# adobe/3D-FM-GAN

Hardware: AMD Instinct MI355X
Metric: (photo,render) pairs/sec (higher is better)
Workload: dtype f32; 1 GPU; pairs1024: cfg4 shard: E_Tsr+E_W+E_W_Plus(18 styles) on 256^2 -> co-mod -> Generator(1024) forward, fp32, B=8/GPU; pairs_per_gpu=8, global_pairs=8, image_size=1024, parallelism=replicas x1 (batch-sharded, no collective), launch=eager, ranks=1, full=False

## Files before the change

### 3d-fm-gan_amd/csrc/conv3x3_x3.hip

```cpp
#include "bf16_mfma.h"

namespace {

enum { C3_NONE = 0, C3_LRELU = 1, C3_PRELU = 2 };

struct C3Params {
  const float* in; const unsigned short* wt; const float* aux; float* out;
  int batch, cin, cout, h, w, oh, ow;
  int tiles_x, tiles_y, o_tiles, mp;
  float alpha;
  int stride, epi;
  int in_nhwc, out_nhwc;
};

template <int S>
struct C3Tile {
  static constexpr int BM = 64, TH = 4, TW = 32;
  static constexpr int PH = S * (TH - 1) + 3, PWP = S * (TW - 1) + 3, EVEN = (PWP + 1) / 2;
  static constexpr int PLANE = PH * PWP;
  static constexpr size_t LDS = (size_t)(3 * 2 * PLANE) * 16;
  static constexpr int BLOCKS_PER_CU = S == 1 ? 3 : 2;
};

bool c3_plan(C3Params& p) {
  if (p.batch <= 0 || p.cin <= 0 || p.cout <= 0 || p.h <= 0 || p.w <= 0) return false;
  if (p.stride != 1 && p.stride != 2) return false;
  if (p.in_nhwc && (p.cin & 3)) return false;
  using Tile = C3Tile<1>;
  p.oh = (p.h - 1) / p.stride + 1; p.ow = (p.w - 1) / p.stride + 1;
  p.mp = (p.cout + 31) / 32 * 32;
  p.tiles_x = (p.ow + Tile::TW - 1) / Tile::TW;
  p.tiles_y = (p.oh + Tile::TH - 1) / Tile::TH;
  p.o_tiles = (p.cout + Tile::BM - 1) / Tile::BM;
  if ((long long)p.cin * p.h * p.w * 4 >= 0xFFFFFFF0LL) return false;
  if ((long long)((p.cin + 15) / 16) * 54 * p.mp * 16 >= 0xFFFFFFF0LL) return false;
  if ((long long)p.o_tiles * p.tiles_x * p.tiles_y * p.batch > 0x7fffffffLL) return false;
  if ((long long)p.batch * p.cout * p.oh * p.ow > (1LL << 40)) return false;
  return true;
}

template <int S, bool NHWC_IN, int EPI>
__global__ __launch_bounds__(256, C3Tile<S>::BLOCKS_PER_CU) void conv3x3_mfma_bf16x3(const C3Params p) {
  using Tile = C3Tile<S>;
  constexpr int BM = Tile::BM, TH = Tile::TH, TW = Tile::TW, PWP = Tile::PWP, EVEN = Tile::EVEN, PLANE = Tile::PLANE;
  constexpr int RNP = 2;
  constexpr bool QUAD = NHWC_IN && S == 2;
  constexpr int NU = QUAD ? (4 * PLANE + 255) / 256 : (PLANE + 255) / 256, NV = QUAD ? 4 : 16;
  static_assert(NU <= 16, "one staging unit per issue_x call");
  extern __shared__ u32x4 smem_q[];
  u32x4* Xs = smem_q;

  const int tid = threadIdx.x, lane = tid & 63, wave = __builtin_amdgcn_readfirstlane(tid >> 6);
  const int l31 = lane & 31, khalf = lane >> 5, wm = wave & 1, wn = wave >> 1;
  const int kq = tid & 3;
  unsigned lb = xcd_remap(blockIdx.x, gridDim.x);
  const int o_tile = lb % p.o_tiles; lb /= p.o_tiles;
  const int tx_i = lb % p.tiles_x; lb /= p.tiles_x;
  const int ty_i = lb % p.tiles_y;
  const int b = lb / p.tiles_y;
  const int o0 = o_tile * BM, x0 = tx_i * TW, y0 = ty_i * TH;
  const int hw = p.h * p.w;
  const float* in_b = p.in + (long long)b * p.cin * hw;

  f32x16 acc[RNP], acc_lo[RNP];
#pragma unroll
  for (int g = 0; g < RNP; ++g)
#pragma unroll
    for (int r = 0; r < 16; ++r) { acc[g][r] = 0.f; acc_lo[g][r] = 0.f; }

  constexpr unsigned PARK = 0xFFFFFFF0u;
  const unsigned x_bytes = (unsigned)((long long)p.cin * hw * 4);
  const unsigned mp16 = (unsigned)p.mp * 16u;
  const unsigned w_bytes = (unsigned)((p.cin + 15) >> 4) * 54u * mp16;
  const auto rsrc_x = __builtin_amdgcn_make_buffer_rsrc(const_cast<float*>(in_b), 0, x_bytes, 0x00020000);
  const auto rsrc_w = __builtin_amdgcn_make_buffer_rsrc(const_cast<unsigned short*>(p.wt), 0, w_bytes, 0x00020000);
  unsigned xvo[NU];
#pragma unroll
  for (int u = 0; u < NU; ++u) {
    const int q = QUAD ? (tid + 256 * u) >> 2 : tid + 256 * u;
    const int r = q / PWP, t = q - r * PWP;
    const int c = S == 1 ? t : (t < EVEN ? 2 * t : 2 * (t - EVEN) + 1);
    const int y = S * y0 + r - 1, x = S * x0 + c - 1;
    const bool inside = q < PLANE && y >= 0 && y < p.h && x >= 0 && x < p.w;
    const unsigned pos_bytes = NHWC_IN ? 4u * (unsigned)p.cin : 4u;
    xvo[u] = inside ? (unsigned)(y * p.w + x) * pos_bytes + (QUAD ? 16u * (unsigned)kq : 0u) : PARK;
  }
  const int arow = o0 + wm * 32 + l31;
  const unsigned avo = arow < p.mp ? (unsigned)(khalf * p.mp + arow) * 16u : PARK;

  float xv[NU][NV];
  auto issue_x = [&](int i0, int kc) {
    if constexpr (QUAD) {
      if (kc < NU) {
// ... 44 lines not shown
          dst[0] = ph; dst[4 * PLANE] = pm; dst[8 * PLANE] = pl;
        }
      }
    } else {
      if (i0 + 16 > p.cin) {
#pragma unroll
        for (int kc = 0; kc < 16; ++kc)
          if (i0 + kc >= p.cin) {
#pragma unroll
            for (int u = 0; u < NU; ++u) xv[u][kc] = 0.f;
          }
      }
#pragma unroll
      for (int u = 0; u < NU; ++u) {
        const int q = tid + 256 * u;
        if (q < PLANE) {
#pragma unroll
          for (int hh = 0; hh < 2; ++hh) {
            unsigned h[4], m[4], l[4];
#pragma unroll
            for (int e = 0; e < 4; ++e) split2(xv[u][8 * hh + 2 * e], xv[u][8 * hh + 2 * e + 1], h[e], m[e], l[e]);
            u32x4 ph = {h[0], h[1], h[2], h[3]}, pm = {m[0], m[1], m[2], m[3]}, pl = {l[0], l[1], l[2], l[3]};
            Xs[(0 * 2 + hh) * PLANE + q] = ph;
            Xs[(1 * 2 + hh) * PLANE + q] = pm;
            Xs[(2 * 2 + hh) * PLANE + q] = pl;
          }
        }
      }
    }
  };

  int pbase[RNP];
#pragma unroll
  for (int g = 0; g < RNP; ++g) pbase[g] = khalf * PLANE + S * (wn * RNP + g) * PWP + l31;

  struct Ops { u32x4 a[3]; bf16x8 b[3][RNP]; };
  auto fetch_a = [&](Ops& o, unsigned soff_chunk, int t) {
#pragma unroll
    for (int pc = 0; pc < 3; ++pc)
      o.a[pc] = __builtin_bit_cast(u32x4, __builtin_amdgcn_raw_buffer_load_b128(rsrc_w, avo, soff_chunk + (unsigned)(pc * 18 + t * 2) * mp16, 0));
  };
  auto fetch_b = [&](Ops& o, int t) {
    const int ky = t / 3, kx = t - 3 * ky;
    const int off = S == 1 ? ky * PWP + kx : ky * PWP + (kx & 1) * EVEN + (kx >> 1);
#pragma unroll
    for (int pc = 0; pc < 3; ++pc)
#pragma unroll
      for (int g = 0; g < RNP; ++g) o.b[pc][g] = __builtin_bit_cast(bf16x8, Xs[pc * 2 * PLANE + pbase[g] + off]);
  };
  unsigned wflag = 0;

  const int chunks = (p.cin + 15) >> 4;
#pragma unroll
  for (int kc = 0; kc < 16; ++kc) issue_x(0, kc);
  for (int ch = 0; ch < chunks; ++ch) {
    const unsigned soff_chunk = (unsigned)ch * 54u * mp16;
    Ops ops[2];
    fetch_a(ops[0], soff_chunk, 0);
    __syncthreads();
    commit_x(16 * ch);
    __syncthreads();
    __builtin_amdgcn_sched_barrier(0);
    fetch_b(ops[0], 0);
    const int i0n = ch + 1 < chunks ? 16 * (ch + 1) : 0;
#pragma unroll
    for (int t = 0; t < 9; ++t) {
      __builtin_amdgcn_sched_barrier(0);
      if (t + 1 < 9) {
        fetch_a(ops[(t + 1) & 1], soff_chunk, t + 1);
        __builtin_amdgcn_sched_barrier(0);
        issue_x(i0n, 2 * t); issue_x(i0n, 2 * t + 1);
        fetch_b(ops[(t + 1) & 1], t + 1);
      }
      __builtin_amdgcn_sched_barrier(0);
      const Ops& o = ops[t & 1];
#pragma unroll
      for (int e = 0; e < 4; ++e) wflag |= ((o.a[0][e] & 0x7f807f80u) + 0x00800080u) & 0x80008000u;
      __builtin_amdgcn_s_setprio(1);
#pragma unroll
      for (int q = 0; q < 6; ++q)
#pragma unroll
        for (int g = 0; g < RNP; ++g) {
          f32x16& dst = q == 5 ? acc[g] : acc_lo[g];
          dst = __builtin_amdgcn_mfma_f32_32x32x16_bf16(__builtin_bit_cast(bf16x8, o.a[PA[q]]), o.b[PB[q]][g], dst, 0, 0, 0);
        }
      __builtin_amdgcn_s_setprio(0);
    }
    __builtin_amdgcn_sched_barrier(0);
  }
#pragma unroll
  for (int g = 0; g < RNP; ++g)
#pragma unroll
    for (int r = 0; r < 16; ++r) acc[g][r] = __fadd_rn(acc[g][r], acc_lo[g][r]);

  float* out_b = p.out + (long long)b * p.cout * p.oh * p.ow;
  const float alpha = p.alpha;
  auto epilogue = [&](float v, float a) -> float {
    if constexpr (EPI == C3_LRELU) {
      const float t = __fadd_rn(v, a);
      return t > 0.f ? t : t * alpha;
    } else if constexpr (EPI == C3_PRELU) {
      return v > 0.f ? v : a * v;
    } else {
      return v;
    }
  };
  const long long ost_o = p.out_nhwc ? 1 : (long long)p.oh * p.ow, ost_p = p.out_nhwc ? p.cout : 1;
  if (__syncthreads_or((xflag != xflag) | (wflag != 0u))) {
    const int pp = tid & 127, oy = y0 + (pp >> 5), ox = x0 + (pp & 31);
    if (oy >= p.oh || ox >= p.ow) return;
    for (int oo = 0; oo < 32; ++oo) {
      const int o = o0 + (tid >> 7) * 32 + oo;
      if (o >= p.cout) return;
      float s = 0.f;
      for (int i = 0; i < p.cin; ++i) {
        const long long slot0 = (long long)(i >> 4) * 54 * p.mp;
        const int hh = (i >> 3) & 1, j = i & 7;
        for (int t = 0; t < 9; ++t) {
          const int y = S * oy + t / 3 - 1, x = S * ox + t % 3 - 1;
          const long long at = NHWC_IN ? (long long)(y * p.w + x) * p.cin + i : (long long)i * hw + y * p.w + x;
          const float xin = (y >= 0 && y < p.h && x >= 0 && x < p.w) ? in_b[at] : 0.f;
          float wv = 0.f;
#pragma unroll
          for (int pc = 0; pc < 3; ++pc)
            wv += bf16_to_f32(p.wt[((slot0 + (long long)(pc * 18 + t * 2 + hh) * p.mp + o) << 3) + j]);
          s = __builtin_fmaf(wv, xin, s);
        }
      }
      out_b[o * ost_o + ((long long)oy * p.ow + ox) * ost_p] = epilogue(s, (EPI != C3_NONE && p.aux) ? p.aux[o] : 0.f);
    }
    return;
  }

  const int orow = o0 + wm * 32 + 4 * khalf;
  float aux_r[16];
#pragma unroll
  for (int r = 0; r < 16; ++r)
    aux_r[r] = (EPI != C3_NONE && p.aux) ? p.aux[min(orow + (r & 3) + 8 * (r >> 2), p.cout - 1)] : 0.f;
#pragma unroll
  for (int g = 0; g < RNP; ++g) {
    const int py_ = y0 + wn * RNP + g, px_ = x0 + l31;
    if (py_ >= p.oh || px_ >= p.ow) continue;
    float* dpos = out_b + ((long long)py_ * p.ow + px_) * ost_p;
    float v[16];
#pragma unroll
    for (int r = 0; r < 16; ++r) v[r] = epilogue(acc[g][r], aux_r[r]);
    if (p.out_nhwc && (p.cout & 3) == 0) {
#pragma unroll
      for (int j = 0; j < 4; ++j) {
        const int o = orow + 8 * j;
        if (o < p.cout) {
          f32x4 q4 = {v[4 * j], v[4 * j + 1], v[4 * j + 2], v[4 * j + 3]};
          *reinterpret_cast<f32x4*>(dpos + o) = q4;
        }
      }
    } else {
#pragma unroll
      for (int r = 0; r < 16; ++r) {
        const int o = orow + (r & 3) + 8 * (r >> 2);
        if (o < p.cout) dpos[o * ost_o] = v[r];
      }
    }
  }
}

template <int S, bool NHWC_IN, int EPI>
int c3_launch(const C3Params& p, hipStream_t s) {
  using Tile = C3Tile<S>;
  void (*kernel)(const C3Params) = conv3x3_mfma_bf16x3<S, NHWC_IN, EPI>;
  static bool opted_in = false;
  opt_in_dynamic_lds(kernel, Tile::LDS, opted_in);
  const long long blocks = (long long)p.o_tiles * p.tiles_x * p.tiles_y * p.batch;
  hipLaunchKernelGGL(kernel, dim3((unsigned)blocks), dim3(256), Tile::LDS, s, p);
  return fmgan_check_launch();
}

template <int S, bool NHWC_IN>
int c3_launch_epi(const C3Params& p, hipStream_t s) {
  if (p.epi == C3_LRELU) return c3_launch<S, NHWC_IN, C3_LRELU>(p, s);
  if (p.epi == C3_PRELU) return c3_launch<S, NHWC_IN, C3_PRELU>(p, s);
  return c3_launch<S, NHWC_IN, C3_NONE>(p, s);
}

int conv3x3_bf16x3(const float* in, const void* wt, const float* aux, float* out, int batch, int cin, int cout, int h, int w,
                   int stride, int in_nhwc, int out_nhwc, int epi, float alpha, hipStream_t s) {
  if (batch < 0 || cin <= 0 || cout <= 0 || h <= 0 || w <= 0 || (stride != 1 && stride != 2)) return FMGAN_EINVAL;
  if ((in_nhwc != 0 && in_nhwc != 1) || (out_nhwc != 0 && out_nhwc != 1) || epi < C3_NONE || epi > C3_PRELU) return FMGAN_EINVAL;
  if (batch == 0) return FMGAN_OK;
  C3Params p{};
  p.in = in; p.wt = (const unsigned short*)wt; p.aux = aux; p.out = out;
  p.batch = batch; p.cin = cin; p.cout = cout; p.h = h; p.w = w; p.alpha = alpha;
  p.stride = stride; p.epi = epi; p.in_nhwc = in_nhwc; p.out_nhwc = out_nhwc;
  if (!c3_plan(p)) return FMGAN_EUNSUPPORTED;
  if (!in || !wt || !out || (epi == C3_PRELU && !aux)) return FMGAN_EINVAL;
  if (in_nhwc && ((uintptr_t)in & 15)) return FMGAN_EINVAL;
  if (out_nhwc && (cout & 3) == 0 && ((uintptr_t)out & 15)) return FMGAN_EINVAL;
  if (stride == 1) return in_nhwc ? c3_launch_epi<1, true>(p, s) : c3_launch_epi<1, false>(p, s);
  return in_nhwc ? c3_launch_epi<2, true>(p, s) : c3_launch_epi<2, false>(p, s);
}

}

extern "C" int fmgan_conv3x3s2_bf16x3_supported(int batch, int cin, int cout, int h, int w) {
  return fmgan_conv3x3_bf16x3_supported(batch, cin, cout, h, w, 2, 0);
}

extern "C" int fmgan_conv3x3s2_bf16x3_f32(const float* in, const void* wt_split, const float* bias, float* out, int batch,
                                          int cin, int cout, int h, int w, float alpha, int out_nhwc, void* stream) {
  return conv3x3_bf16x3(in, wt_split, bias, out, batch, cin, cout, h, w, 2, 0, out_nhwc, C3_LRELU, alpha, (hipStream_t)stream);
}

extern "C" int fmgan_conv3x3_bf16x3_supported(int batch, int cin, int cout, int h, int w, int stride, int in_nhwc) {
  C3Params p{};
  p.batch = batch; p.cin = cin; p.cout = cout; p.h = h; p.w = w; p.stride = stride; p.in_nhwc = in_nhwc;
  return c3_plan(p) ? 1 : 0;
}

extern "C" int fmgan_conv3x3_bf16x3_f32(const float* in, const void* wt_split, const float* aux, float* out, int batch,
                                        int cin, int cout, int h, int w, int stride, int in_nhwc, int out_nhwc,
                                        int epilogue, float alpha, void* stream) {
  return conv3x3_bf16x3(in, wt_split, aux, out, batch, cin, cout, h, w, stride, in_nhwc, out_nhwc, epilogue, alpha,
                        (hipStream_t)stream);
}
```

### 3d-fm-gan_amd/op/_native/__init__.py

```python
from .core import (
    LIB_PATH, F32, F64, F16, BF16, FMGAN_OK, FMGAN_EINVAL, FMGAN_EUNSUPPORTED, amp_fwd, amp_bwd, lib, check, served,
    require_gpu, dtype_code, ptr, fp, require_f32_gpu, on_device, nhwc_dense, set_observer, launching)
from .activation import (
    activation_io, current_activation_io, io16, amp_fwd_io, BLUR_PATHS, upfirdn2d_out_size, upfirdn2d,
    upfirdn2d_strided, blur_noise_bias_act_serves, blur_noise_bias_act, fused_bias_act, fused_bias_act_backward,
    noise_bias_act, prelu_backward, dtype16_code, upfirdn2d16, fused_bias_act16, fused_bias_act16_backward)
from .conv import (
    modconv_demod, modconv_wsq, modconv_weight_prep, aligned_rows_shape, aligned_rows_buffer, modconv_precision,
    current_modconv_precision, modconv2d, modconv2d_rgb_fusable, modconv2d_select, modconv2d_tiles, modconv2d_rgb,
    modconv_weight_to_bf16, modconv_weight_to_bf16x3, conv_weight_to_bf16x3, conv3x3s2_bf16x3_supported,
    conv3x3s2_bf16x3, conv3x3_bf16x3_supported, conv3x3_bf16x3, C3_EPILOGUES, modconv_wgrad, wino_weight,
    wino_input, wino_output, modconv2d_winograd, torgb,
    torgb_backward, equal_linear, style_bank, style_bank_concat, demod_bank)
from .encoder import bn_prelu, se_pool, se_gate, ir_tail
from .loss import (
    LPIPS_SIZE, face_region_loss, face_region_loss_backward, render_mask, lpips_distance, lpips_distance_backward,
    lpips_pair_input, projection_loss_fwd, projection_loss_bwd, HEATMAP_SIZE, face_crop_serves, face_crop_fwd,
    face_crop_bwd, detector_input, heatmap_distance_serves, heatmap_distance_fwd, heatmap_distance_bwd,
    landmark_decode)
from .evaluation import (
    face_input_pool, face_input, f64p, fid_stats_serves, fid_stats_update, fid_stats_finish, INCEPTION_SIZE,
    inception_input)
from .image import (
    images_to_tensor, resize_output_size, resize_plan, resize_images, tensor_to_images, tiles_to_canvas,
    BANK_GATHER_BANKS, BANK_GATHER_GROUPS, bank_gather)
from .optim import (
    lbfgs_segments, lbfgs_pair, lbfgs_coeffs, lbfgs_direction, lbfgs_update, lbfgs_gather, EMA_CHUNK,
    LOSS_ROW_COLUMNS, ema_blocks, ema, loss_row)
```

### 3d-fm-gan_amd/op/_native/conv.py

```python
import ctypes

import torch

from .core import ambient, check, fp, launching, lib, nhwc_dense, _noise_args, on_device, ptr, require_gpu, served


def modconv_demod(weight, style, scale, eps=1e-8, wsq=None):
    cout, cin, kh, kw = weight.shape[-4:]
    style = style.contiguous()
    demod = torch.empty((style.shape[0], cout), dtype=torch.float32, device=style.device)
    with on_device(style) as stream:
        if wsq is not None:
            check(lib().fmgan_modconv_demod_wsq_f32(fp(wsq), fp(style), fp(demod), style.shape[0], cout, cin,
                                                    float(scale), float(eps), stream), 'modconv_demod_wsq')
        else:
            check(lib().fmgan_modconv_demod_f32(fp(weight), fp(style), fp(demod), style.shape[0], cout, cin,
                                                kh * kw, float(scale), float(eps), stream), 'modconv_demod')
    return demod


def modconv_wsq(weight):
    cout, cin, kh, kw = weight.shape[-4:]
    wsq = torch.empty((cout, cin), dtype=torch.float32, device=weight.device)
    with on_device(weight) as stream:
# ... 100 lines not shown
    rgb = torch.empty((b, rgb_c, h, w), dtype=torch.float32, device=x.device)
    nz, nb = _noise_args(noise)
    sk = rgb_skip.contiguous() if rgb_skip is not None else None
    wmod = torch.empty((b, 3, cout), dtype=torch.float32, device=x.device)
    with on_device(x) as stream:
        check(lib().fmgan_torgb_weight_mod_f32(fp(rgb_weight), fp(rgb_style), fp(wmod), b, cout, rgb_c,
                                               float(rgb_scale), stream), 'torgb_weight_mod')
    with launching(x, 'modconv2d', (b, cin, cout, h, w, 0)) as stream:
        st = lib().fmgan_modconv2d_rgb_f32(fp(x), fp(wt), fp(style), fp(demod), fp(out), b, cin, cout, h, w,
                                           fp(nz), fp(noise_weight), fp(bias), nb, 1, float(alpha), float(act_scale),
                                           fp(wmod), fp(rgb_bias), fp(sk), fp(rgb), rgb_c, stream)
    check(st, 'modconv2d_rgb')
    return out, rgb


def modconv_weight_to_bf16(wt):
    cin, taps, cout = wt.shape
    nbytes = lib().fmgan_modconv_weight_bf16_bytes(cin, cout, taps)
    wtb = torch.empty(nbytes // 2, dtype=torch.int16, device=wt.device)
    with on_device(wt) as stream:
        check(lib().fmgan_modconv_weight_to_bf16(fp(wt), ptr(wtb), cin, cout, taps, stream), 'modconv_weight_to_bf16')
    return wtb


def modconv_weight_to_bf16x3(wt):
    cin, taps, cout = wt.shape
    nbytes = lib().fmgan_modconv_weight_bf16x3_bytes(cin, cout, taps)
    wts = torch.empty(nbytes // 2, dtype=torch.int16, device=wt.device)
    with on_device(wt) as stream:
        check(lib().fmgan_modconv_weight_to_bf16x3(fp(wt), ptr(wts), cin, cout, taps, stream), 'modconv_weight_to_bf16x3')
    return wts


def conv_weight_to_bf16x3(weight):
    require_gpu(weight, 'weight')
    cout, cin, kh, kw = weight.shape
    with launching(weight, 'conv_weight_bf16x3', (cout, cin, kh * kw)):
        wt = weight.detach().permute(1, 2, 3, 0).reshape(cin, kh * kw, cout).contiguous()
        return modconv_weight_to_bf16x3(wt)


def conv3x3s2_bf16x3_supported(batch, cin, cout, h, w):
    return bool(lib().fmgan_conv3x3s2_bf16x3_supported(int(batch), int(cin), int(cout), int(h), int(w)))


def conv3x3s2_bf16x3(x, wts, bias, cout, alpha=0.01, channels_last=False):
    require_gpu(x, 'input')
    in_nhwc = _c3_input_layout('conv3x3s2_bf16x3', x)
    b, cin, h, w = x.shape
    out = torch.empty((b, cout, (h - 1) // 2 + 1, (w - 1) // 2 + 1), dtype=torch.float32, device=x.device,
                      memory_format=torch.channels_last if channels_last else torch.contiguous_format)
    with launching(x, 'conv3x3s2_bf16x3', (b, cin, cout, h, w)) as stream:
        if in_nhwc:
            st = lib().fmgan_conv3x3_bf16x3_f32(fp(x), ptr(wts), fp(bias), fp(out), b, cin, cout, h, w, 2, 1,
                                                int(bool(channels_last)), C3_EPILOGUES['lrelu'], float(alpha), stream)
        else:
            st = lib().fmgan_conv3x3s2_bf16x3_f32(fp(x), ptr(wts), fp(bias), fp(out), b, cin, cout, h, w, float(alpha),
                                                  int(bool(channels_last)), stream)
    return out if served(st, 'conv3x3s2_bf16x3') else None


C3_EPILOGUES = {None: 0, 'lrelu': 1, 'prelu': 2}


def _c3_input_layout(what, x):
    if x.is_contiguous():
        return 0
    if nhwc_dense(x):
        return 1
    raise RuntimeError(f'{what}: input must be NCHW-contiguous or dense channels_last, got strides {x.stride()}')


def conv3x3_bf16x3_supported(batch, cin, cout, h, w, stride=1, channels_last_in=False):
    return bool(lib().fmgan_conv3x3_bf16x3_supported(int(batch), int(cin), int(cout), int(h), int(w), int(stride),
                                                     int(bool(channels_last_in))))


def conv3x3_bf16x3(x, wts, cout, stride=1, epilogue=None, aux=None, alpha=0.01, channels_last=False):
    require_gpu(x, 'input')
    in_nhwc = _c3_input_layout('conv3x3_bf16x3', x)
    epi = C3_EPILOGUES[epilogue]
    if epilogue == 'prelu' and (aux is None or aux.numel() != cout):
        raise RuntimeError('conv3x3_bf16x3: the prelu epilogue needs one slope per output channel')
    if aux is not None:
        aux = aux.contiguous()
    stride = int(stride)
    b, cin, h, w = x.shape
    out = torch.empty((b, cout, (h - 1) // max(stride, 1) + 1, (w - 1) // max(stride, 1) + 1), dtype=torch.float32,
                      device=x.device, memory_format=torch.channels_last if channels_last else torch.contiguous_format)
    with launching(x, 'conv3x3_bf16x3', (b, cin, cout, h, w, stride, epi)) as stream:
        st = lib().fmgan_conv3x3_bf16x3_f32(fp(x), ptr(wts), fp(aux), fp(out), b, cin, cout, h, w, stride, in_nhwc,
                                            int(bool(channels_last)), epi, float(alpha), stream)
    return out if served(st, 'conv3x3_bf16x3') else None


def modconv_wgrad(go, demod, x, style, scale, fast_only=False, mode=0):
    go, x, style = go.contiguous(), x.contiguous(), style.contiguous()
    b, cout = go.shape[:2]
    cin, h, w = x.shape[1:]
    if (fast_only or mode != 0) and (cin < 48 or cout < 48):
        return None
    ws_bytes = lib().fmgan_modconv_wgrad_mode_workspace_bytes(b, cin, cout, h, w, int(mode))
    if ws_bytes == 0:
        return None
    ws = torch.empty(ws_bytes // 4, dtype=torch.float32, device=x.device)
    gw = torch.empty((cout, cin, 3, 3), dtype=torch.float32, device=x.device)
    with launching(x, 'modconv_wgrad', (b, cin, cout, h, w, int(mode))) as stream:
        st = lib().fmgan_modconv_wgrad_mode_f32(fp(go), fp(demod), fp(x), fp(style), fp(gw), b, cin, cout, h, w,
                                                int(mode), float(scale), fp(ws), ws_bytes, stream)
    check(st, 'modconv_wgrad')
    return gw


def wino_weight(wt):
    cin, taps, cout = wt.shape
    if taps != 9:
        raise RuntimeError('wino_weight: 3x3 weights only')
    u = torch.empty((16, cout, cin), dtype=torch.float32, device=wt.device)
    with on_device(wt) as stream:
        check(lib().fmgan_wino_weight_f32(fp(wt), fp(u), cin, cout, stream), 'wino_weight')
    return u


def wino_input(x, style):
    require_gpu(x, 'input')
    x, style = x.contiguous(), style.contiguous()
# ... 118 lines not shown
```

### 3d-fm-gan_amd/op/_native/core.py

```python
import ctypes
import os

import torch

_PKG = os.path.dirname(os.path.dirname(os.path.dirname(os.path.abspath(__file__))))
LIB_PATH = os.environ.get('FMGAN_LIB') or os.path.join(_PKG, 'csrc', 'libfmgan_hip.so')

F32, F64, F16 = 0, 1, 2
BF16 = 3
FMGAN_OK, FMGAN_EINVAL, FMGAN_EUNSUPPORTED = 0, -1, -2
_DTYPES = {torch.float32: F32, torch.float64: F64, torch.float16: F16}

_lib = None

amp_fwd = torch.amp.custom_fwd(device_type='cuda', cast_inputs=torch.float32)
amp_bwd = torch.amp.custom_bwd(device_type='cuda')


class ambient:
    values, text, scope, var = (), '', None, ''

    def __init__(self, value):
        if value not in self.values:
            raise ValueError(self.text)
# ... 38 lines not shown
    _sig(L.fmgan_noise_bias_act_f32, [vp] * 5 + [i] * 4 + [f, f, vp])
    _sig(L.fmgan_fused_bias_act_bwd_blocks, [ll, i])
    _sig(L.fmgan_fused_bias_act_bwd_f32, [vp] * 4 + [ll, i, f, f, vp])
    _sig(L.fmgan_prelu_backward_blocks, [ll, i])
    _sig(L.fmgan_prelu_backward_f32, [vp] * 5 + [ll, i, vp])
    _sig(L.fmgan_act16_fba_select, [i, ll, i, i, i, i])
    _sig(L.fmgan_act16_fba, [i, vp, vp, vp, vp, ll, i, i, i, i, f, f, vp])
    _sig(L.fmgan_act16_fba_bwd_blocks, [ll, i])
    _sig(L.fmgan_act16_fba_bwd, [i] + [vp] * 4 + [ll, i, f, f, vp])
    _sig(L.fmgan_ufd16_select, [i] * 15)
    _sig(L.fmgan_ufd16, [i, vp, vp, vp] + [i] * 14 + [vp])
    _sig(L.fmgan_modconv_demod_f32, [vp] * 3 + [i] * 4 + [f, f, vp])
    _sig(L.fmgan_modconv_wsq_f32, [vp] * 2 + [i] * 3 + [vp])
    _sig(L.fmgan_modconv_demod_wsq_f32, [vp] * 3 + [i] * 3 + [f, f, vp])
    _sig(L.fmgan_modconv_weight_prep_f32, [vp, vp, i, i, i, f, i, vp])
    _sig(L.fmgan_modconv2d_workspace_bytes, [i] * 6, ll)
    _sig(L.fmgan_modconv2d_f32, [vp] * 5 + [i] * 6 + [vp] * 3 + [i, i, f, f, ll, i, vp, ll, vp])
    _sig(L.fmgan_modconv2d_rgb_fusable, [i] * 5)
    _sig(L.fmgan_modconv2d_select, [i] * 8 + [ctypes.POINTER(i)] * 5)
    _sig(L.fmgan_modconv2d_tiles, [ctypes.POINTER(i), i])
    _sig(L.fmgan_modconv2d_rgb_f32, [vp] * 5 + [i] * 5 + [vp] * 3 + [i, i, f, f] + [vp] * 4 + [i, vp])
    _sig(L.fmgan_modconv_weight_bf16_bytes, [i] * 3, ll)
    _sig(L.fmgan_modconv_weight_to_bf16, [vp, vp, i, i, i, vp])
    _sig(L.fmgan_modconv2d_bf16_supported, [i] * 6)
    _sig(L.fmgan_modconv2d_bf16, [vp] * 5 + [i] * 6 + [vp] * 3 + [i, i, f, f, ll, i, vp])
    _sig(L.fmgan_modconv_weight_bf16x3_bytes, [i] * 3, ll)
    _sig(L.fmgan_modconv_weight_to_bf16x3, [vp, vp, i, i, i, vp])
    _sig(L.fmgan_modconv2d_bf16x3_supported, [i] * 6)
    _sig(L.fmgan_modconv2d_bf16x3, [vp] * 5 + [i] * 6 + [vp] * 3 + [i, i, f, f, ll, i, vp])
    _sig(L.fmgan_conv3x3s2_bf16x3_supported, [i] * 5)
    _sig(L.fmgan_conv3x3s2_bf16x3_f32, [vp] * 4 + [i] * 5 + [f, i, vp])
    _sig(L.fmgan_conv3x3_bf16x3_supported, [i] * 7)
    _sig(L.fmgan_conv3x3_bf16x3_f32, [vp] * 4 + [i] * 9 + [f, vp])
    _sig(L.fmgan_modconv_wgrad_workspace_bytes, [i] * 5, ll)
    _sig(L.fmgan_modconv_wgrad_f32, [vp] * 5 + [i] * 5 + [f, vp, ll, vp])
    _sig(L.fmgan_modconv_wgrad_mode_workspace_bytes, [i] * 6, ll)
    _sig(L.fmgan_modconv_wgrad_mode_f32, [vp] * 5 + [i] * 6 + [f, vp, ll, vp])
    _sig(L.fmgan_wino_weight_f32, [vp, vp, i, i, vp])
    _sig(L.fmgan_wino_input_f32, [vp] * 3 + [i] * 4 + [vp])
    _sig(L.fmgan_wino_output_f32, [vp] * 6 + [i] * 6 + [f, f, vp])
    _sig(L.fmgan_torgb_weight_mod_f32, [vp] * 3 + [i] * 3 + [f, vp])
    _sig(L.fmgan_torgb_f32, [vp] * 6 + [i] * 4 + [f, vp])
    _sig(L.fmgan_torgb_backward_splits, [i] * 3)
    _sig(L.fmgan_torgb_backward_f32, [vp] * 6 + [i] * 4 + [f, vp])
    _sig(L.fmgan_equal_linear_f32, [vp] * 4 + [i] * 3 + [vp])
    _sig(L.fmgan_style_bank_entry_bytes, [])
    _sig(L.fmgan_style_bank_f32, [vp, i, vp, vp, i, i, i, vp, vp])
    _sig(L.fmgan_style_bank_concat_f32, [vp, i, vp, vp, i, i, i, i, vp, vp])
    _sig(L.fmgan_demod_bank_f32, [vp, i, vp, i, vp, vp])
    _sig(L.fmgan_weight_refresh_blocks, [i, i, i, i, ll], ll)
    _sig(L.fmgan_weight_refresh_f32, [vp, i, ll, vp])
    _sig(L.fmgan_bn_prelu_f32, [vp] * 5 + [f, vp, vp] + [vp] * 4 + [f, vp, vp] + [i] * 5 + [vp])
    _sig(L.fmgan_se_pool_chunks, [i] * 4)
    _sig(L.fmgan_se_pool_f32, [vp, vp] + [i] * 4 + [vp])
    _sig(L.fmgan_se_gate_f32, [vp, i, ll] + [vp] * 4 + [f] + [vp] * 3 + [i] * 3 + [vp])
    _sig(L.fmgan_ir_tail_f32, [vp] * 5 + [f, vp, vp] + [i] * 3 + [vp] * 4 + [f, vp] + [vp] * 4 + [f, vp] + [i] * 4 + [vp])
    _sig(L.fmgan_face_region_blocks, [i, ll])
    _sig(L.fmgan_face_region_loss_f32, [vp] * 3 + [i, i, ll, vp])
    _sig(L.fmgan_face_region_backward_f32, [vp] * 4 + [i, i, ll, vp])
    _sig(L.fmgan_render_mask_f32, [vp] * 2 + [i, i, ll, vp])
    _sig(L.fmgan_lpips_distance_blocks, [i] * 3)
    _sig(L.fmgan_lpips_distance_f32, [vp] * 4 + [i, i, i, f, vp])
    _sig(L.fmgan_lpips_distance_backward_f32, [vp] * 6 + [i, i, i, f, vp])
    _sig(L.fmgan_lpips_pair_input_select, [i] * 8)
    _sig(L.fmgan_lpips_pair_input_f32, [vp] * 5 + [i] * 8 + [vp])
    _sig(L.fmgan_projection_loss_select, [i] * 4)
# ... 160 lines not shown
```

### 3d-fm-gan_amd/op/live_weights.py

```python
import weakref

import numpy as np
import torch

from . import _native

_ENTRY = np.dtype([('src', '<u8'), ('dst', '<u8'), ('dst2', '<u8'), ('n', '<i8'), ('kind', '<i4'), ('cout', '<i4'),
                   ('cin', '<i4'), ('ktaps', '<i4'), ('scale', '<f4'), ('block_begin', '<u4')])


def _check_layout():
    if _native.lib().fmgan_refresh_entry_bytes() != _ENTRY.itemsize:
        raise RuntimeError('fmgan_refresh_entry layout mismatch between libfmgan_hip.so and op/live_weights.py')


class LiveWeights:

    def __init__(self, root):
        self.root = root
        self.active = False
        self._key = None
        self._table = None
        self._blocks = 0
        self._n = 0
# ... 67 lines not shown
            _native.check(_native.lib().fmgan_weight_refresh_f32(self._table.data_ptr(), self._n, self._blocks, stream),
                          'weight_refresh')
        return True

    def fresh(self):
        return _Fresh(self)


class _Fresh:
    def __init__(self, lw):
        self.lw = lw

    def __enter__(self):
        self.prev = self.lw.active
        if not self.prev:
            self.lw.active = self.lw.refresh()
        return self.lw

    def __exit__(self, *exc):
        self.lw.active = self.prev
        return False


def live(module):
    lv = getattr(module, '_live', None)
    if lv is not None and lv[0].active and not torch.is_grad_enabled():
        return lv[1], lv[2]
    return None


_SPLIT = weakref.WeakKeyDictionary()


def split_conv_weight(conv):
    w = conv.weight
    key = (w.data_ptr(), w._version, w.device, tuple(w.shape), tuple(w.stride()))
    kept = _SPLIT.get(conv)
    stream = torch.cuda.current_stream(w.device)
    if kept is None or kept[0] != key:
        img = _native.conv_weight_to_bf16x3(w)
        built = torch.cuda.Event()
        built.record(stream)
        kept = (key, img, built, stream)
        _SPLIT[conv] = kept
    elif kept[3] != stream:
        stream.wait_event(kept[2])
    return kept[1]


def drop_split_weight(conv=None):
    if conv is None:
        _SPLIT.clear()
    else:
        _SPLIT.pop(conv, None)
```

### 3d-fm-gan_amd/psp_encoder_model/encoders/psp_encoders.py

```python
import math
import os

import torch
import torch.nn.functional as F
from torch import nn
from torch.nn import BatchNorm2d, Conv2d, Module, Sequential

from . import helpers
from .helpers import PReLU, bottleneck_IR, bottleneck_IR_SE, get_blocks
from stylegan2 import EqualLinear
from op import fused_leaky_relu
from op import _native
from op.live_weights import LiveWeights, split_conv_weight
from Util.streams import overlap_ok, run_deferred, side_streams

HEAD_STREAMS = int(os.environ.get('FMGAN_PSP_STREAMS', '2'))
GROUP_HEADS = os.environ.get('FMGAN_PSP_GROUPED', '0') == '1'

HEADS_X3 = os.environ.get('FMGAN_PSP_HEADS_X3', '1') == '1'
X3_MIN_OUT = 32
X3_TAIL_CHANNELS_LAST = True
X3_HEAD_CHANNELS_LAST_IN = True

_TAPS = {18: (3, 5, 7), 50: (6, 20, 23)}


class GradualStyleBlock(Module):

    def __init__(self, in_c, out_c, spatial):
        super().__init__()
        self.out_c = out_c
        self.spatial = spatial
        layers, c = [], in_c
        for _ in range(int(math.log2(spatial))):
            layers += [Conv2d(c, out_c, kernel_size=3, stride=2, padding=1), nn.LeakyReLU()]
            c = out_c
        self.convs = nn.Sequential(*layers)
        self.linear = EqualLinear(out_c, out_c, lr_mul=1)

    def x3_serves(self, x):
        if not (HEADS_X3 and x.is_cuda and x.dtype == torch.float32 and not torch.is_grad_enabled()):
            return False
        conv = self.convs[0]
        if conv.weight.dtype != torch.float32 or conv.bias is None or (x.shape[3] - 1) // 2 + 1 < X3_MIN_OUT:
            return False
        return _native.conv3x3s2_bf16x3_supported(x.shape[0], conv.in_channels, conv.out_channels, x.shape[2], x.shape[3])

    @staticmethod
    def x3_reads(x):
        return X3_HEAD_CHANNELS_LAST_IN and _native.nhwc_dense(x) and x.shape[1] % 4 == 0

    def _first_x3(self, x):
        conv, act = self.convs[0], self.convs[1]
        y = _native.conv3x3s2_bf16x3(x, split_conv_weight(conv), conv.bias, conv.out_channels, act.negative_slope,
                                     channels_last=X3_TAIL_CHANNELS_LAST)
        if y is None:
            raise RuntimeError('conv3x3s2_bf16x3 declined a shape its query accepted')
        return y

    def forward(self, x, x_nchw=None):
        if x.is_cuda and x.dtype == torch.float32:
            convs = list(zip(self.convs[0::2], self.convs[1::2]))
            if self.x3_serves(x):
                if x_nchw is None:
                    x_nchw = x if self.x3_reads(x) else x.contiguous()
                x = self._first_x3(x_nchw)
                convs = convs[1:]
            for conv, act in convs:
                y = F.conv2d(x, conv.weight, None, conv.stride, conv.padding)
                if y.is_contiguous(memory_format=torch.channels_last) and not y.is_contiguous():
                    n, c, h, w = y.shape
                    y = fused_leaky_relu(y.permute(0, 2, 3, 1).reshape(-1, c), conv.bias, act.negative_slope, 1.0)
                    x = y.view(n, h, w, c).permute(0, 3, 1, 2)
                else:
                    x = fused_leaky_relu(y, conv.bias, act.negative_slope, 1.0)
            return self.linear(x.reshape(-1, self.out_c))
        return self.linear(self.convs(x).reshape(-1, self.out_c))


class GradualStyleEncoder(Module):
    def __init__(self, num_layers, mode='ir', opts=None):
        super().__init__()
        assert num_layers in [18, 50, 100, 152], 'num_layers should be 18, 50, 100, or 152'
        assert mode in ['ir', 'ir_se'], 'mode should be ir or ir_se'
        self.num_layers = num_layers
        unit = bottleneck_IR if mode == 'ir' else bottleneck_IR_SE
        self.input_layer = Sequential(Conv2d(opts.input_nc, 64, (3, 3), 1, 1, bias=False), BatchNorm2d(64), PReLU(64))
        self.body = Sequential(*[unit(b.in_channel, b.depth, b.stride) for stage in get_blocks(num_layers) for b in stage])
        self.style_count = opts.n_styles
        self.coarse_ind = 3
        self.middle_ind = 7
        self.styles = nn.ModuleList()
        for i in range(self.style_count):
            spatial = 16 if i < self.coarse_ind else (32 if i < self.middle_ind else 64)
            self.styles.append(GradualStyleBlock(512, 512, spatial))
        self.latlayer1 = nn.Conv2d(256, 512, kernel_size=1, stride=1, padding=0)
        self.latlayer2 = nn.Conv2d(128, 512, kernel_size=1, stride=1, padding=0)
        self.channels_last = True
        self._cl_key = None
        self._live_weights = None
        self._flat = None
# ... 138 lines not shown
```

### include/fmgan_hip.h

```cpp
#ifndef FMGAN_HIP_H
#define FMGAN_HIP_H

#ifdef __cplusplus
extern "C" {
#endif

#define FMGAN_ABI_VERSION 1

#define FMGAN_OK            0
#define FMGAN_EINVAL       -1
#define FMGAN_EUNSUPPORTED -2
#define FMGAN_ELAUNCH      -3
#define FMGAN_EOVERFLOW    -4

#define FMGAN_F32 0
#define FMGAN_F64 1
#define FMGAN_F16 2
#define FMGAN_BF16 3

int         fmgan_abi_version(void);
const char *fmgan_status_string(int status);

int fmgan_upfirdn2d_select(int dtype, int major, int in_h, int in_w, int minor,
                           int kernel_h, int kernel_w, int up_x, int up_y,
// ... 182 lines not shown
                        int batch, int cin, int cout, int h, int w, int mode,
                        const float *noise, const float *noise_weight, const float *bias,
                        int noise_batch, int fuse_act, float alpha, float act_scale,
                        long long out_plane_stride, int out_row_stride,
                        void *workspace, long long workspace_bytes, void *stream);

long long fmgan_modconv_weight_bf16_bytes(int cin, int cout, int ktaps);
int fmgan_modconv_weight_to_bf16(const float *wt, void *wt_bf16, int cin, int cout, int ktaps, void *stream);
int fmgan_modconv2d_bf16_supported(int batch, int cin, int cout, int h, int w, int mode);
int fmgan_modconv2d_bf16(const float *in, const void *wt_bf16, const float *style, const float *demod, float *out,
                         int batch, int cin, int cout, int h, int w, int mode,
                         const float *noise, const float *noise_weight, const float *bias,
                         int noise_batch, int fuse_act, float alpha, float act_scale,
                         long long out_plane_stride, int out_row_stride, void *stream);

long long fmgan_modconv_weight_bf16x3_bytes(int cin, int cout, int ktaps);
int fmgan_modconv_weight_to_bf16x3(const float *wt, void *wt_split, int cin, int cout, int ktaps, void *stream);
int fmgan_modconv2d_bf16x3_supported(int batch, int cin, int cout, int h, int w, int mode);
int fmgan_modconv2d_bf16x3(const float *in, const void *wt_split, const float *style, const float *demod, float *out,
                           int batch, int cin, int cout, int h, int w, int mode,
                           const float *noise, const float *noise_weight, const float *bias,
                           int noise_batch, int fuse_act, float alpha, float act_scale,
                           long long out_plane_stride, int out_row_stride, void *stream);

int fmgan_conv3x3s2_bf16x3_supported(int batch, int cin, int cout, int h, int w);
int fmgan_conv3x3s2_bf16x3_f32(const float *in, const void *wt_split, const float *bias, float *out,
                               int batch, int cin, int cout, int h, int w, float alpha, int out_nhwc, void *stream);

int fmgan_conv3x3_bf16x3_supported(int batch, int cin, int cout, int h, int w, int stride, int in_nhwc);
int fmgan_conv3x3_bf16x3_f32(const float *in, const void *wt_split, const float *aux, float *out,
                             int batch, int cin, int cout, int h, int w, int stride, int in_nhwc, int out_nhwc,
                             int epilogue, float alpha, void *stream);

int fmgan_torgb_weight_mod_f32(const float *rgb_weight, const float *rgb_style, float *wmod,
                               int batch, int cout, int rgb_channels, float rgb_scale, void *stream);
int fmgan_modconv2d_rgb_fusable(int batch, int cin, int cout, int h, int w);
int fmgan_modconv2d_rgb_f32(const float *in, const float *wt, const float *style,
                            const float *demod, float *out,
                            int batch, int cin, int cout, int h, int w,
                            const float *noise, const float *noise_weight, const float *bias,
                            int noise_batch, int fuse_act, float alpha, float act_scale,
                            const float *rgb_wmod, const float *rgb_bias,
                            const float *rgb_skip, float *rgb_out, int rgb_channels, void *stream);

int fmgan_modconv2d_select(int batch, int cin, int cout, int h, int w, int mode, int rgb, int has_workspace,
                           int *cfg, int *variant, int *bm, int *bn, int *ksplit);
int fmgan_modconv2d_tiles(int *out, int cap);

long long fmgan_modconv_wgrad_workspace_bytes(int batch, int cin, int cout, int h, int w);
long long fmgan_modconv_wgrad_mode_workspace_bytes(int batch, int cin, int cout, int h, int w, int mode);
int fmgan_modconv_wgrad_mode_f32(const float *go, const float *demod, const float *x, const float *style,
                                 float *gw, int batch, int cin, int cout, int h, int w, int mode, float scale,
                                 void *workspace, long long workspace_bytes, void *stream);
int fmgan_modconv_wgrad_f32(const float *go, const float *demod, const float *x, const float *style,
                            float *gw, int batch, int cin, int cout, int h, int w, float scale,
                            void *workspace, long long workspace_bytes, void *stream);

int fmgan_torgb_f32(const float *in, const float *weight, const float *style,
                    const float *bias, const float *skip, float *out,
                    int batch, int cin, int cout, int hw, float scale, void *stream);

int fmgan_torgb_backward_splits(int batch, int cin, int hw);
int fmgan_torgb_backward_f32(const float *x, const float *grad_out, const float *weight, const float *style,
                             float *grad_x, float *m_partial, int batch, int cin, int cout, int hw, float scale,
                             void *stream);

// ... 65 lines not shown
```

Measured before the change: 425.9 pairs/s.

## Add narrow-tile bf16x3 conv kernel for small-spatial pSp encoder tail convs

Parameterizes the bf16x3 MFMA 3x3 conv tile by width, output-channel block, rows-per-wave and a weight-fetch ring depth. It then instantiates a stride-2 NHWC LReLU tail kernel with 16- or 8-wide tiles and a nine-deep weight prefetch ring. The pSp encoder style-map convs on small feature maps now use it instead of F.conv2d plus a separate activation. The aim is to fit tiles to the tiny spatial sizes, fuse bias and activation, and hide weight-load latency. In exchange it adds more template instantiations and register pressure from the deep ring.

```diff
diff --git a/3d-fm-gan_amd/csrc/conv3x3_x3.hip b/3d-fm-gan_amd/csrc/conv3x3_x3.hip
--- a/3d-fm-gan_amd/csrc/conv3x3_x3.hip
+++ b/3d-fm-gan_amd/csrc/conv3x3_x3.hip
@@ -13,20 +13,24 @@
   int in_nhwc, out_nhwc;
 };
 
-template <int S>
+template <int S, int TW_ = 32, int BM_ = 64, int RNP_ = 2, int A_RING_ = 0>
 struct C3Tile {
-  static constexpr int BM = 64, TH = 4, TW = 32;
+  static constexpr int BM = BM_, TW = TW_, RNP = RNP_, A_RING = A_RING_;
+  static_assert(A_RING == 0 || 9 % A_RING == 0, "a tap keeps its ring slot from chunk to chunk");
+  static constexpr int WM = BM / 32, WN = 4 / WM, RPG = 32 / TW, TH = WN * RNP * RPG;
+  static constexpr int TW_LOG2 = TW == 32 ? 5 : TW == 16 ? 4 : 3, NPOS = TH * TW, NPOS_LOG2 = NPOS == 128 ? 7 : 6;
+  static_assert((WM == 1 || WM == 2) && (TW == 32 || TW == 16 || TW == 8) && (NPOS == 128 || NPOS == 64), "tile");
   static constexpr int PH = S * (TH - 1) + 3, PWP = S * (TW - 1) + 3, EVEN = (PWP + 1) / 2;
   static constexpr int PLANE = PH * PWP;
   static constexpr size_t LDS = (size_t)(3 * 2 * PLANE) * 16;
   static constexpr int BLOCKS_PER_CU = S == 1 ? 3 : 2;
 };
 
-bool c3_plan(C3Params& p) {
+template <class Tile>
+bool c3_plan_tile(C3Params& p) {
   if (p.batch <= 0 || p.cin <= 0 || p.cout <= 0 || p.h <= 0 || p.w <= 0) return false;
   if (p.stride != 1 && p.stride != 2) return false;
   if (p.in_nhwc && (p.cin & 3)) return false;
-  using Tile = C3Tile<1>;
   p.oh = (p.h - 1) / p.stride + 1; p.ow = (p.w - 1) / p.stride + 1;
   p.mp = (p.cout + 31) / 32 * 32;
   p.tiles_x = (p.ow + Tile::TW - 1) / Tile::TW;
@@ -38,12 +42,12 @@
   if ((long long)p.batch * p.cout * p.oh * p.ow > (1LL << 40)) return false;
   return true;
 }
-
-template <int S, bool NHWC_IN, int EPI>
-__global__ __launch_bounds__(256, C3Tile<S>::BLOCKS_PER_CU) void conv3x3_mfma_bf16x3(const C3Params p) {
-  using Tile = C3Tile<S>;
-  constexpr int BM = Tile::BM, TH = Tile::TH, TW = Tile::TW, PWP = Tile::PWP, EVEN = Tile::EVEN, PLANE = Tile::PLANE;
-  constexpr int RNP = 2;
+bool c3_plan(C3Params& p) { return c3_plan_tile<C3Tile<1>>(p); }
+
+template <class Tile, int S, bool NHWC_IN, int EPI>
+__device__ __forceinline__ void c3_block(const C3Params p) {
+  constexpr int BM = Tile::BM, TW = Tile::TW, PWP = Tile::PWP, EVEN = Tile::EVEN, PLANE = Tile::PLANE;
+  constexpr int RNP = Tile::RNP, RPG = Tile::RPG, WM = Tile::WM;
   constexpr bool QUAD = NHWC_IN && S == 2;
   constexpr int NU = QUAD ? (4 * PLANE + 255) / 256 : (PLANE + 255) / 256, NV = QUAD ? 4 : 16;
   static_assert(NU <= 16, "one staging unit per issue_x call");
@@ -51,14 +55,15 @@
   u32x4* Xs = smem_q;
 
   const int tid = threadIdx.x, lane = tid & 63, wave = __builtin_amdgcn_readfirstlane(tid >> 6);
-  const int l31 = lane & 31, khalf = lane >> 5, wm = wave & 1, wn = wave >> 1;
+  const int l31 = lane & 31, khalf = lane >> 5, wm = wave & (WM - 1), wn = wave >> (WM - 1);
+  const int lr = l31 >> Tile::TW_LOG2, lc = l31 & (TW - 1);
   const int kq = tid & 3;
   unsigned lb = xcd_remap(blockIdx.x, gridDim.x);
   const int o_tile = lb % p.o_tiles; lb /= p.o_tiles;
   const int tx_i = lb % p.tiles_x; lb /= p.tiles_x;
   const int ty_i = lb % p.tiles_y;
   const int b = lb / p.tiles_y;
-  const int o0 = o_tile * BM, x0 = tx_i * TW, y0 = ty_i * TH;
+  const int o0 = o_tile * BM, x0 = tx_i * TW, y0 = ty_i * Tile::TH;
   const int hw = p.h * p.w;
   const float* in_b = p.in + (long long)b * p.cin * hw;
 
@@ -169,7 +174,7 @@
 
   int pbase[RNP];
 #pragma unroll
-  for (int g = 0; g < RNP; ++g) pbase[g] = khalf * PLANE + S * (wn * RNP + g) * PWP + l31;
+  for (int g = 0; g < RNP; ++g) pbase[g] = khalf * PLANE + S * ((wn * RNP + g) * RPG + lr) * PWP + lc;
 
   struct Ops { u32x4 a[3]; bf16x8 b[3][RNP]; };
   auto fetch_a = [&](Ops& o, unsigned soff_chunk, int t) {
@@ -190,6 +195,47 @@
   const int chunks = (p.cin + 15) >> 4;
 #pragma unroll
   for (int kc = 0; kc < 16; ++kc) issue_x(0, kc);
+  if constexpr (Tile::A_RING != 0) {
+    constexpr int AR = Tile::A_RING, AD = AR - 1;
+    Ops ring[AR];
+#pragma unroll
+    for (int t = 0; t < AD; ++t) fetch_a(ring[t], 0u, t);
+    for (int ch = 0; ch < chunks; ++ch) {
+      const unsigned soff_chunk = (unsigned)ch * 54u * mp16;
+      const unsigned soff_next = ch + 1 < chunks ? soff_chunk + 54u * mp16 : 0u;
+      __syncthreads();
+      commit_x(16 * ch);
+      __syncthreads();
+      __builtin_amdgcn_sched_barrier(0);
+      fetch_b(ring[0], 0);
+      const int i0n = ch + 1 < chunks ? 16 * (ch + 1) : 0;
+#pragma unroll
+      for (int t = 0; t < 9; ++t) {
+        __builtin_amdgcn_sched_barrier(0);
+        fetch_a(ring[(t + AD) % AR], t + AD < 9 ? soff_chunk : soff_next, (t + AD) % 9);
+        __builtin_amdgcn_sched_barrier(0);
+        if (t == 0) {
+#pragma unroll
+          for (int kc = 0; kc < 16; ++kc) issue_x(i0n, kc);
+        }
+        if (t + 1 < 9) fetch_b(ring[(t + 1) & 1], t + 1);
+        __builtin_amdgcn_sched_barrier(0);
+        const Ops &oa = ring[t % AR], &ob = ring[t & 1];
+#pragma unroll
+        for (int e = 0; e < 4; ++e) wflag |= ((oa.a[0][e] & 0x7f807f80u) + 0x00800080u) & 0x80008000u;
+        __builtin_amdgcn_s_setprio(1);
+#pragma unroll
+        for (int q = 0; q < 6; ++q)
+#pragma unroll
+          for (int g = 0; g < RNP; ++g) {
+            f32x16& dst = q == 5 ? acc[g] : acc_lo[g];
+            dst = __builtin_amdgcn_mfma_f32_32x32x16_bf16(__builtin_bit_cast(bf16x8, oa.a[PA[q]]), ob.b[PB[q]][g], dst, 0, 0, 0);
+          }
+        __builtin_amdgcn_s_setprio(0);
+      }
+      __builtin_amdgcn_sched_barrier(0);
+    }
+  } else
   for (int ch = 0; ch < chunks; ++ch) {
     const unsigned soff_chunk = (unsigned)ch * 54u * mp16;
     Ops ops[2];
@@ -244,10 +290,11 @@
   };
   const long long ost_o = p.out_nhwc ? 1 : (long long)p.oh * p.ow, ost_p = p.out_nhwc ? p.cout : 1;
   if (__syncthreads_or((xflag != xflag) | (wflag != 0u))) {
-    const int pp = tid & 127, oy = y0 + (pp >> 5), ox = x0 + (pp & 31);
+    constexpr int CPT = BM * Tile::NPOS / 256;
+    const int pp = tid & (Tile::NPOS - 1), oy = y0 + (pp >> Tile::TW_LOG2), ox = x0 + (pp & (TW - 1));
     if (oy >= p.oh || ox >= p.ow) return;
-    for (int oo = 0; oo < 32; ++oo) {
-      const int o = o0 + (tid >> 7) * 32 + oo;
+    for (int oo = 0; oo < CPT; ++oo) {
+      const int o = o0 + (tid >> Tile::NPOS_LOG2) * CPT + oo;
       if (o >= p.cout) return;
       float s = 0.f;
       for (int i = 0; i < p.cin; ++i) {
@@ -276,7 +323,7 @@
     aux_r[r] = (EPI != C3_NONE && p.aux) ? p.aux[min(orow + (r & 3) + 8 * (r >> 2), p.cout - 1)] : 0.f;
 #pragma unroll
   for (int g = 0; g < RNP; ++g) {
-    const int py_ = y0 + wn * RNP + g, px_ = x0 + l31;
+    const int py_ = y0 + (wn * RNP + g) * RPG + lr, px_ = x0 + lc;
     if (py_ >= p.oh || px_ >= p.ow) continue;
     float* dpos = out_b + ((long long)py_ * p.ow + px_) * ost_p;
     float v[16];
@@ -302,14 +349,44 @@
 }
 
 template <int S, bool NHWC_IN, int EPI>
-int c3_launch(const C3Params& p, hipStream_t s) {
-  using Tile = C3Tile<S>;
-  void (*kernel)(const C3Params) = conv3x3_mfma_bf16x3<S, NHWC_IN, EPI>;
-  static bool opted_in = false;
+__global__ __launch_bounds__(256, C3Tile<S>::BLOCKS_PER_CU) void conv3x3_mfma_bf16x3(const C3Params p) {
+  c3_block<C3Tile<S>, S, NHWC_IN, EPI>(p);
+}
+
+template <int TW> struct TailTile { using type = C3Tile<2, TW, 64, 1, 9>; };
+
+template <int TW>
+__global__ __launch_bounds__(256, 2) void conv3x3_tail_x3(const C3Params p) {
+  c3_block<typename TailTile<TW>::type, 2, true, C3_LRELU>(p);
+}
+
+template <class Tile>
+int c3_launch_kernel(void (*kernel)(const C3Params), bool& opted_in, const C3Params& p, hipStream_t s) {
   opt_in_dynamic_lds(kernel, Tile::LDS, opted_in);
   const long long blocks = (long long)p.o_tiles * p.tiles_x * p.tiles_y * p.batch;
   hipLaunchKernelGGL(kernel, dim3((unsigned)blocks), dim3(256), Tile::LDS, s, p);
   return fmgan_check_launch();
+}
+
+template <int S, bool NHWC_IN, int EPI>
+int c3_launch(const C3Params& p, hipStream_t s) {
+  static bool opted_in = false;
+  return c3_launch_kernel<C3Tile<S>>(conv3x3_mfma_bf16x3<S, NHWC_IN, EPI>, opted_in, p, s);
+}
+
+template <int TW>
+int tail_launch(const C3Params& p, hipStream_t s) {
+  static bool opted_in = false;
+  return c3_launch_kernel<typename TailTile<TW>::type>(conv3x3_tail_x3<TW>, opted_in, p, s);
+}
+
+int tail_plan(C3Params& p) {
+  if (p.batch <= 0 || p.cin <= 0 || p.cout <= 0 || p.h <= 0 || p.w <= 0) return FMGAN_EINVAL;
+  p.stride = 2; p.epi = C3_LRELU; p.in_nhwc = 1;
+  const int ow = (p.w - 1) / 2 + 1;
+  if (ow > 16 || ow <= 4) return FMGAN_EUNSUPPORTED;
+  if (ow > 8) return c3_plan_tile<TailTile<16>::type>(p) ? 16 : FMGAN_EUNSUPPORTED;
+  return c3_plan_tile<TailTile<8>::type>(p) ? 8 : FMGAN_EUNSUPPORTED;
 }
 
 template <int S, bool NHWC_IN>
@@ -359,3 +436,22 @@
   return conv3x3_bf16x3(in, wt_split, aux, out, batch, cin, cout, h, w, stride, in_nhwc, out_nhwc, epilogue, alpha,
                         (hipStream_t)stream);
 }
+
+extern "C" int fmgan_conv3x3_tail_bf16x3_select(int batch, int cin, int cout, int h, int w) {
+  C3Params p{};
+  p.batch = batch; p.cin = cin; p.cout = cout; p.h = h; p.w = w;
+  return tail_plan(p);
+}
+
+extern "C" int fmgan_conv3x3_tail_bf16x3_f32(const float* in, const void* wt_split, const float* bias, float* out, int batch,
+                                             int cin, int cout, int h, int w, float alpha, int out_nhwc, void* stream) {
+  if (out_nhwc != 0 && out_nhwc != 1) return FMGAN_EINVAL;
+  C3Params p{};
+  p.in = in; p.wt = (const unsigned short*)wt_split; p.aux = bias; p.out = out;
+  p.batch = batch; p.cin = cin; p.cout = cout; p.h = h; p.w = w; p.alpha = alpha; p.out_nhwc = out_nhwc;
+  const int tw = tail_plan(p);
+  if (tw < 0) return tw;
+  if (!in || !wt_split || !out) return FMGAN_EINVAL;
+  if (((uintptr_t)in & 15) || (out_nhwc && (cout & 3) == 0 && ((uintptr_t)out & 15))) return FMGAN_EINVAL;
+  return tw == 16 ? tail_launch<16>(p, (hipStream_t)stream) : tail_launch<8>(p, (hipStream_t)stream);
+}
diff --git a/3d-fm-gan_amd/op/_native/__init__.py b/3d-fm-gan_amd/op/_native/__init__.py
--- a/3d-fm-gan_amd/op/_native/__init__.py
+++ b/3d-fm-gan_amd/op/_native/__init__.py
@@ -9,7 +9,8 @@
     modconv_demod, modconv_wsq, modconv_weight_prep, aligned_rows_shape, aligned_rows_buffer, modconv_precision,
     current_modconv_precision, modconv2d, modconv2d_rgb_fusable, modconv2d_select, modconv2d_tiles, modconv2d_rgb,
     modconv_weight_to_bf16, modconv_weight_to_bf16x3, conv_weight_to_bf16x3, conv3x3s2_bf16x3_supported,
-    conv3x3s2_bf16x3, conv3x3_bf16x3_supported, conv3x3_bf16x3, C3_EPILOGUES, modconv_wgrad, wino_weight,
+    conv3x3s2_bf16x3, conv3x3_bf16x3_supported, conv3x3_bf16x3, C3_EPILOGUES, conv3x3_tail_bf16x3_select,
+    conv3x3_tail_bf16x3, modconv_wgrad, wino_weight,
     wino_input, wino_output, modconv2d_winograd, torgb,
     torgb_backward, equal_linear, style_bank, style_bank_concat, demod_bank)
 from .encoder import bn_prelu, se_pool, se_gate, ir_tail
diff --git a/3d-fm-gan_amd/op/_native/conv.py b/3d-fm-gan_amd/op/_native/conv.py
--- a/3d-fm-gan_amd/op/_native/conv.py
+++ b/3d-fm-gan_amd/op/_native/conv.py
@@ -156,10 +156,10 @@
     return wts
 
 
-def conv_weight_to_bf16x3(weight):
+def conv_weight_to_bf16x3(weight, bracket='conv_weight_bf16x3'):
     require_gpu(weight, 'weight')
     cout, cin, kh, kw = weight.shape
-    with launching(weight, 'conv_weight_bf16x3', (cout, cin, kh * kw)):
+    with launching(weight, bracket, (cout, cin, kh * kw)):
         wt = weight.detach().permute(1, 2, 3, 0).reshape(cin, kh * kw, cout).contiguous()
         return modconv_weight_to_bf16x3(wt)
 
@@ -216,6 +216,23 @@
         st = lib().fmgan_conv3x3_bf16x3_f32(fp(x), ptr(wts), fp(aux), fp(out), b, cin, cout, h, w, stride, in_nhwc,
                                             int(bool(channels_last)), epi, float(alpha), stream)
     return out if served(st, 'conv3x3_bf16x3') else None
+
+
+def conv3x3_tail_bf16x3_select(batch, cin, cout, h, w):
+    return int(lib().fmgan_conv3x3_tail_bf16x3_select(int(batch), int(cin), int(cout), int(h), int(w)))
+
+
+def conv3x3_tail_bf16x3(x, wts, bias, cout, alpha=0.01, channels_last=True):
+    require_gpu(x, 'input')
+    if not nhwc_dense(x):
+        raise RuntimeError(f'conv3x3_tail_bf16x3: input must be dense channels_last, got strides {x.stride()}')
+    b, cin, h, w = x.shape
+    out = torch.empty((b, cout, (h - 1) // 2 + 1, (w - 1) // 2 + 1), dtype=torch.float32, device=x.device,
+                      memory_format=torch.channels_last if channels_last else torch.contiguous_format)
+    with launching(x, 'conv3x3_tail_bf16x3', (b, cin, cout, h, w)) as stream:
+        st = lib().fmgan_conv3x3_tail_bf16x3_f32(fp(x), ptr(wts), fp(bias), fp(out), b, cin, cout, h, w, float(alpha),
+                                                 int(bool(channels_last)), stream)
+    return out if served(st, 'conv3x3_tail_bf16x3') else None
 
 
 def modconv_wgrad(go, demod, x, style, scale, fast_only=False, mode=0):
diff --git a/3d-fm-gan_amd/op/_native/core.py b/3d-fm-gan_amd/op/_native/core.py
--- a/3d-fm-gan_amd/op/_native/core.py
+++ b/3d-fm-gan_amd/op/_native/core.py
@@ -94,6 +94,8 @@
     _sig(L.fmgan_conv3x3s2_bf16x3_f32, [vp] * 4 + [i] * 5 + [f, i, vp])
     _sig(L.fmgan_conv3x3_bf16x3_supported, [i] * 7)
     _sig(L.fmgan_conv3x3_bf16x3_f32, [vp] * 4 + [i] * 9 + [f, vp])
+    _sig(L.fmgan_conv3x3_tail_bf16x3_select, [i] * 5)
+    _sig(L.fmgan_conv3x3_tail_bf16x3_f32, [vp] * 4 + [i] * 5 + [f, i, vp])
     _sig(L.fmgan_modconv_wgrad_workspace_bytes, [i] * 5, ll)
     _sig(L.fmgan_modconv_wgrad_f32, [vp] * 5 + [i] * 5 + [f, vp, ll, vp])
     _sig(L.fmgan_modconv_wgrad_mode_workspace_bytes, [i] * 6, ll)
diff --git a/3d-fm-gan_amd/op/live_weights.py b/3d-fm-gan_amd/op/live_weights.py
--- a/3d-fm-gan_amd/op/live_weights.py
+++ b/3d-fm-gan_amd/op/live_weights.py
@@ -123,13 +123,13 @@
 _SPLIT = weakref.WeakKeyDictionary()
 
 
-def split_conv_weight(conv):
+def split_conv_weight(conv, bracket='conv_weight_bf16x3'):
     w = conv.weight
     key = (w.data_ptr(), w._version, w.device, tuple(w.shape), tuple(w.stride()))
     kept = _SPLIT.get(conv)
     stream = torch.cuda.current_stream(w.device)
     if kept is None or kept[0] != key:
-        img = _native.conv_weight_to_bf16x3(w)
+        img = _native.conv_weight_to_bf16x3(w, bracket)
         built = torch.cuda.Event()
         built.record(stream)
         kept = (key, img, built, stream)
diff --git a/3d-fm-gan_amd/psp_encoder_model/encoders/psp_encoders.py b/3d-fm-gan_amd/psp_encoder_model/encoders/psp_encoders.py
--- a/3d-fm-gan_amd/psp_encoder_model/encoders/psp_encoders.py
+++ b/3d-fm-gan_amd/psp_encoder_model/encoders/psp_encoders.py
@@ -21,6 +21,9 @@
 X3_MIN_OUT = 32
 X3_TAIL_CHANNELS_LAST = True
 X3_HEAD_CHANNELS_LAST_IN = True
+
+TAIL_X3 = os.environ.get('FMGAN_PSP_TAIL_X3', '1') == '1'
+TAIL_X3_WIDTHS = (16,)
 
 _TAPS = {18: (3, 5, 7), 50: (6, 20, 23)}
 
@@ -58,6 +61,15 @@
             raise RuntimeError('conv3x3s2_bf16x3 declined a shape its query accepted')
         return y
 
+    @staticmethod
+    def tail_x3_serves(x, conv):
+        if not (TAIL_X3 and x.is_cuda and x.dtype == torch.float32 and not torch.is_grad_enabled()):
+            return False
+        if conv.weight.dtype != torch.float32 or conv.bias is None or not _native.nhwc_dense(x):
+            return False
+        return _native.conv3x3_tail_bf16x3_select(x.shape[0], conv.in_channels, conv.out_channels, x.shape[2],
+                                                  x.shape[3]) in TAIL_X3_WIDTHS
+
     def forward(self, x, x_nchw=None):
         if x.is_cuda and x.dtype == torch.float32:
             convs = list(zip(self.convs[0::2], self.convs[1::2]))
@@ -67,6 +79,12 @@
                 x = self._first_x3(x_nchw)
                 convs = convs[1:]
             for conv, act in convs:
+                if self.tail_x3_serves(x, conv):
+                    x = _native.conv3x3_tail_bf16x3(x, split_conv_weight(conv, 'conv_tail_weight_bf16x3'), conv.bias,
+                                                    conv.out_channels, act.negative_slope)
+                    if x is None:
+                        raise RuntimeError('conv3x3_tail_bf16x3 declined a shape its query accepted')
+                    continue
                 y = F.conv2d(x, conv.weight, None, conv.stride, conv.padding)
                 if y.is_contiguous(memory_format=torch.channels_last) and not y.is_contiguous():
                     n, c, h, w = y.shape
diff --git a/include/fmgan_hip.h b/include/fmgan_hip.h
--- a/include/fmgan_hip.h
+++ b/include/fmgan_hip.h
@@ -238,6 +238,10 @@
                              int batch, int cin, int cout, int h, int w, int stride, int in_nhwc, int out_nhwc,
                              int epilogue, float alpha, void *stream);
 
+int fmgan_conv3x3_tail_bf16x3_select(int batch, int cin, int cout, int h, int w);
+int fmgan_conv3x3_tail_bf16x3_f32(const float *in, const void *wt_split, const float *bias, float *out,
+                                  int batch, int cin, int cout, int h, int w, float alpha, int out_nhwc, void *stream);
+
 int fmgan_torgb_weight_mod_f32(const float *rgb_weight, const float *rgb_style, float *wmod,
                                int batch, int cout, int rgb_channels, float rgb_scale, void *stream);
 int fmgan_modconv2d_rgb_fusable(int batch, int cin, int cout, int h, int w);
```

Result: faster. 433.5 pairs/s, median of 6 (+1.8%).
